# HKUST-Aerial-Robotics/A-LOAM

Measured on AMD Instinct MI355X. Metric: HDL-64 scans/sec (whole node), higher is better.
Workload: dtype f32 features / f64 solve

## Files before the change

### a-loam_amd/binding.py

```python
from __future__ import annotations

import ctypes as C
import os
import re
import subprocess

import numpy as np

from .records import *

_HERE = os.path.dirname(os.path.abspath(__file__))
_ROOT = os.path.dirname(_HERE)
LIB_PATH = os.path.join(_HERE, "lib", "libaloam_mi355x.so")
HEADER_PATH = os.path.join(_ROOT, "include", "aloam_mi355x.h")

MAP_INFO_KEYS = ("cenW", "cenH", "cenD", "frame_count", "from_map_corner", "from_map_surf", "corner_stack", "surf_stack",
                 "corner_num0", "corner_num1", "surf_num0", "surf_num1", "lm_iterations0", "lm_iterations1", "termination0", "compactions")


class AloamError(RuntimeError):
    def __init__(self, code, msg):
        super().__init__(f"aloam error {code}: {msg}")
        self.code = code

# ... 33 lines not shown
        L.aloam_create.argtypes = [C.POINTER(AloamConfig), C.POINTER(vp)]
        L.aloam_create_stages.argtypes = [C.POINTER(AloamConfig), C.c_int, C.POINTER(vp)]
        L.aloam_destroy.argtypes = [vp]; L.aloam_destroy.restype = None
        L.aloam_last_error.argtypes = [vp]; L.aloam_last_error.restype = C.c_char_p
        L.aloam_stream.argtypes = [vp]; L.aloam_stream.restype = vp
        L.aloam_synchronize.argtypes = [vp]
        L.aloam_set_voxel_sum_order.argtypes = [vp, C.c_int]
        L.aloam_scan_register.argtypes = [vp, C.POINTER(vp), ip, C.c_int]
        L.aloam_scan_register_device.argtypes = [vp, vp, C.c_longlong, ip, C.c_int]
        L.aloam_scan_register_host.argtypes = [vp, vp, C.c_longlong, ip, C.c_int]
        L.aloam_process_host.argtypes = [vp, vp, C.c_longlong, ip, C.c_int]
        L.aloam_input_consumed.argtypes = [vp]
        L.aloam_odometry_step.argtypes = [vp]
        L.aloam_process_device.argtypes = [vp, vp, C.c_longlong, ip, C.c_int]
        L.aloam_set_range_decoder.argtypes = [vp, C.POINTER(AloamRangeDecoder)]
        L.aloam_scan_register_range_device.argtypes = [vp, vp, C.c_longlong, ip]
        L.aloam_scan_register_range_host.argtypes = [vp, vp, C.c_longlong, ip]
        L.aloam_process_range_device.argtypes = [vp, vp, C.c_longlong, ip]
        L.aloam_process_range_host.argtypes = [vp, vp, C.c_longlong, ip]
        L.aloam_cloud_size.argtypes = [vp, C.c_int, C.c_int]
        L.aloam_get_cloud.argtypes = [vp, C.c_int, C.c_int, vp, C.c_int]
        L.aloam_get_pose.argtypes = [vp, C.c_int, vp, vp, vp, vp]
        L.aloam_get_odom_stats.argtypes = [vp, C.c_int, C.POINTER(AloamOdomStats)]
        L.aloam_set_features.argtypes = [vp, C.c_int, vp, C.c_int, vp, C.c_int, vp, C.c_int, vp, C.c_int]
        L.aloam_set_last.argtypes = [vp, C.c_int, vp, C.c_int, vp, C.c_int]
        L.aloam_set_state.argtypes = [vp, C.c_int, vp, vp, vp, vp]
        L.aloam_set_system_inited.argtypes = [vp, C.c_int]
        L.aloam_set_active.argtypes = [vp, vp]
        L.aloam_reset_sequences.argtypes = [vp, vp, C.c_int]
        L.aloam_set_map_frozen.argtypes = [vp, vp]
        L.aloam_score_map_corrections.argtypes = [vp, vp, C.c_int, vp, C.c_int, vp, vp]
        L.aloam_apply_map_corrections.argtypes = [vp, vp, C.c_int, vp, C.c_int, vp]
        L.aloam_map_spill_enable.argtypes = [vp, C.c_int, C.c_int]
        L.aloam_export_map_spill.argtypes = [vp, vp, C.c_int, vp, C.c_longlong, vp, C.c_longlong, vp, C.c_int]
        L.aloam_get_map_spill_info.argtypes = [vp, C.c_int, vp]
        L.aloam_atlas_load.argtypes = [vp, vp, C.c_longlong, vp, C.c_longlong]
        L.aloam_atlas_attach.argtypes = [vp, vp]
        L.aloam_atlas_info.argtypes = [vp, vp]
        L.aloam_places_enable.argtypes = [vp, C.c_int, C.c_float, C.c_float]
        L.aloam_places_add.argtypes = [vp, vp, C.c_int]
        L.aloam_places_match.argtypes = [vp, vp, C.c_int, vp, C.c_int, vp]
        L.aloam_places_export.argtypes = [vp, C.c_int, C.c_int, vp]
        L.aloam_places_load.argtypes = [vp, vp, C.c_int]
        L.aloam_places_clear.argtypes = [vp]
        L.aloam_places_info.argtypes = [vp, vp]
        L.aloam_save_sequences.argtypes = [vp, vp, C.c_int, vp, C.c_longlong, vp]
        L.aloam_load_sequences.argtypes = [vp, vp, C.c_int, vp, vp]
        L.aloam_get_ring_ranges.argtypes = [vp, C.c_int, vp, vp]
        L.aloam_get_curvature.argtypes = [vp, C.c_int, vp, C.c_int]
        L.aloam_get_labels.argtypes = [vp, C.c_int, vp, C.c_int]
        L.aloam_get_last_cloud_order.argtypes = [vp, C.c_int, vp]
        if hasattr(L, "aloam_get_solve_lds"):
            L.aloam_get_solve_lds.argtypes = [vp, vp]
        L.aloam_get_correspondences.argtypes = [vp, C.c_int, vp, C.c_int, ip, vp, vp, C.c_int, ip, vp]
        L.aloam_mapping_enable.argtypes = [vp, C.c_float, C.c_float, C.c_int]
        L.aloam_mapping_step.argtypes = [vp]
        L.aloam_mapping_set_pool_limit.argtypes = [vp, C.c_int]
        L.aloam_get_map_pool_info.argtypes = [vp, vp]
        L.aloam_set_map.argtypes = [vp, C.c_int, C.c_int, vp, vp, C.c_int, vp]
        L.aloam_set_map_frame.argtypes = [vp, C.c_int, vp, vp, vp, C.c_int]
        L.aloam_set_full_cloud.argtypes = [vp, C.c_int, vp, C.c_int]
        L.aloam_get_map_pose.argtypes = [vp, C.c_int, vp, vp, vp, vp]
        L.aloam_get_map_info.argtypes = [vp, C.c_int, vp]
        L.aloam_map_cube_counts.argtypes = [vp, C.c_int, C.c_int, vp]
        L.aloam_get_map_cube.argtypes = [vp, C.c_int, C.c_int, C.c_int, vp, C.c_int]
        L.aloam_get_map_cloud.argtypes = [vp, C.c_int, C.c_int, vp, C.c_int]
        L.aloam_export_poses.argtypes = [vp, vp]
        L.aloam_export_clouds.argtypes = [vp, vp, C.c_int, vp, C.c_longlong, vp]
        L.aloam_export_pose_information.argtypes = [vp, C.c_int, vp, C.c_int, vp]
        L.aloam_get_map_factors.argtypes = [vp, C.c_int, vp, C.c_int, ip, vp, C.c_int, ip]
        L.aloam_graph_default_options.argtypes = [C.POINTER(AloamGraphOptions)]; L.aloam_graph_default_options.restype = None
        L.aloam_graph_enable.argtypes = [vp, C.c_int, C.c_int]
        L.aloam_graph_add_nodes.argtypes = [vp, vp, C.c_int, vp]
        L.aloam_graph_add_edges.argtypes = [vp, vp, C.c_int]
        L.aloam_graph_export.argtypes = [vp, C.c_int, C.c_int, C.c_int, vp]
        L.aloam_graph_export_edges.argtypes = [vp, C.c_int, C.c_int, C.c_int, vp]
        L.aloam_graph_clear.argtypes = [vp, vp, C.c_int]
        L.aloam_graph_info.argtypes = [vp, C.c_int, vp]
        L.aloam_graph_optimize.argtypes = [vp, vp, C.c_int, C.POINTER(AloamGraphOptions), vp]
        L.aloam_graph_keyframes_enable.argtypes = [vp, C.c_int, C.c_int]
        L.aloam_graph_export_keyframes.argtypes = [vp, C.c_int, C.c_int, C.c_int, C.c_int, vp, C.c_longlong, vp]
        L.aloam_graph_keyframe_info.argtypes = [vp, C.c_int, vp]
        L.aloam_graph_export_map.argtypes = [vp, vp, C.c_int, vp, C.c_longlong, vp, C.c_longlong, vp, vp]
        L.aloam_graph_apply.argtypes = [vp, vp, C.c_int, vp]
        L.aloam_graph_loop_default_options.argtypes = [C.POINTER(AloamGraphLoopOptions)]; L.aloam_graph_loop_default_options.restype = None
        L.aloam_graph_loops_enable.argtypes = [vp, C.c_int, C.c_int, C.c_int]
        L.aloam_graph_register_loops.argtypes = [vp, vp, C.c_int, C.POINTER(AloamGraphLoopOptions), vp]
        L.aloam_graph_loop_export_target.argtypes = [vp, C.c_int, C.c_int, vp, C.c_longlong, vp]
        L.aloam_graph_loop_default_search.argtypes = [C.POINTER(AloamGraphLoopSearch)]; L.aloam_graph_loop_default_search.restype = None
        L.aloam_graph_search_loops.argtypes = [vp, vp, C.c_int, C.POINTER(AloamGraphLoopSearch), C.POINTER(AloamGraphLoopOptions), vp, vp, vp]
        L.aloam_graph_marginal_default_options.argtypes = [C.POINTER(AloamGraphMarginalOptions)]; L.aloam_graph_marginal_default_options.restype = None
        L.aloam_graph_marginals.argtypes = [vp, vp, C.c_int, C.POINTER(AloamGraphMarginalOptions), vp]
        L.aloam_graph_robust_default_options.argtypes = [C.POINTER(AloamGraphRobustOptions)]; L.aloam_graph_robust_default_options.restype = None
        L.aloam_graph_optimize_robust.argtypes = [vp, vp, C.c_int, C.POINTER(AloamGraphOptions), C.POINTER(AloamGraphRobustOptions), vp, vp, C.c_longlong]
        if hasattr(L, "aloam_graph_propose_loops"):
            L.aloam_graph_propose_loops.argtypes = [vp, vp, C.c_int, C.c_int, C.c_double, C.c_double, C.c_int, C.c_int, C.c_int, C.c_int, vp, vp, vp]
        L.aloam_graph_save.argtypes = [vp, vp, C.c_int, vp, C.c_longlong, vp]
        L.aloam_graph_load.argtypes = [vp, vp, C.c_int, vp, vp]
        L.aloam_profile_enable.argtypes = [vp, C.c_int]
        L.aloam_profile_kernel_count.argtypes = []
        L.aloam_profile_kernel_name.argtypes = [C.c_int]; L.aloam_profile_kernel_name.restype = C.c_char_p
        L.aloam_profile_get.argtypes = [vp, C.c_int, C.POINTER(C.c_double), C.POINTER(C.c_longlong), C.POINTER(C.c_double)]
        _lib = L
    return _lib


# ... 589 lines not shown

    def graph_load(self, slots, blob, offsets):
        ids = _ids(slots)
        off = np.ascontiguousarray(offsets, dtype=np.int64)
        ptr = blob.data_ptr() if hasattr(blob, "data_ptr") else blob.ctypes.data
        self._graph_load_keep = (blob, off)
        self._check(lib().aloam_graph_load(self.h, _ids_arg(ids), len(ids), _vp(ptr), _p(off)))

    def save_sequences_into(self, seqs, dst_ptr, cap_bytes, offsets_ptr):
        ids = _ids(seqs)
        self._check(lib().aloam_save_sequences(self.h, _ids_arg(ids), len(ids), _vp(dst_ptr), int(cap_bytes), _vp(offsets_ptr)))

    def save_sequences(self, seqs, pinned=True):
        import torch
        off = torch.zeros(len(seqs) + 1, dtype=torch.int64, pin_memory=True)
        self.save_sequences_into(seqs, 0, 0, off.data_ptr())
        self.synchronize()
        total = int(off[-1])
        blob = torch.empty(max(total, 16), dtype=torch.uint8, **_where(pinned))
        self.save_sequences_into(seqs, blob.data_ptr(), total, off.data_ptr())
        self.synchronize()
        return (blob[:total].numpy() if pinned else blob[:total]), off.numpy().copy()

    def load_sequences(self, slots, blob, offsets):
        ids = _ids(slots)
        off = np.ascontiguousarray(offsets, dtype=np.int64)
        ptr = blob.data_ptr() if hasattr(blob, "data_ptr") else blob.ctypes.data
        self._load_keep = (blob, off)
        self._check(lib().aloam_load_sequences(self.h, _ids_arg(ids), len(ids), _vp(ptr), _p(off)))

    def odometry_step(self):
        self._check(lib().aloam_odometry_step(self.h))

    def pose(self, seq=0):
        qw, tw, ql, tl = np.zeros(4), np.zeros(3), np.zeros(4), np.zeros(3)
        self._check(lib().aloam_get_pose(self.h, seq, _p(qw), _p(tw), _p(ql), _p(tl)))
        return {"q_w": qw, "t_w": tw, "q_lc": ql, "t_lc": tl}

    def odom_stats(self, seq=0):
        st = AloamOdomStats()
        self._check(lib().aloam_get_odom_stats(self.h, seq, C.byref(st)))
        return {k: list(getattr(st, k)) for k, _ in AloamOdomStats._fields_}

    def last_cloud_order(self, seq=0):
        v = np.zeros(2, np.int32)
        self._check(lib().aloam_get_last_cloud_order(self.h, seq, _p(v)))
        return int(v[0]), int(v[1])

    def solve_lds(self):
        v = np.zeros(3, np.int32)
        self._check(lib().aloam_get_solve_lds(self.h, _p(v)))
        return int(v[0]), int(v[1]), int(v[2])

    def correspondences(self, seq=0):
        cap_e, cap_p = self.n_scans * 12, self.n_scans * 24
        e = np.zeros((cap_e, 9), np.float32); p = np.zeros((cap_p, 12), np.float32)
        eq = np.zeros(cap_e, np.int32); pq = np.zeros(cap_p, np.int32)
        ne, npl = C.c_int(0), C.c_int(0)
        self._check(lib().aloam_get_correspondences(self.h, seq, _p(e), cap_e, C.byref(ne), _p(eq), _p(p), cap_p, C.byref(npl), _p(pq)))
        return e[:ne.value].copy(), p[:npl.value].copy(), eq[:ne.value].copy(), pq[:npl.value].copy()

    def mapping_enable(self, line_res=0.4, plane_res=0.8, pool_points=262144, pool_limit=None):
        if pool_limit is not None:
            self._check(lib().aloam_mapping_set_pool_limit(self.h, int(pool_limit)))
        self._check(lib().aloam_mapping_enable(self.h, float(line_res), float(plane_res), int(pool_points)))

    def map_pool_info(self):
        v = np.zeros(4, np.int32)
        self._check(lib().aloam_get_map_pool_info(self.h, _p(v)))
        return {"pool_points": int(v[0]), "growths": int(v[1]), "limit": int(v[2]), "live_max": int(v[3])}

    def set_map(self, cubes, cls, seq=0):
        ids = np.array(sorted(cubes), np.int32)
        cnt = np.array([len(cubes[int(i)]) for i in ids], np.int32)
        pts = _f32(np.concatenate([cubes[int(i)] for i in ids])) if len(ids) else np.zeros((0, 4), np.float32)
        self._check(lib().aloam_set_map(self.h, seq, cls, _p(ids), _p(cnt), len(ids), _p(pts)))

    def set_map_frame(self, cen, q_wmap_wodom, t_wmap_wodom, frame_count, seq=0):
        a, q, t = np.ascontiguousarray(cen, dtype=np.int32), _f64(q_wmap_wodom), _f64(t_wmap_wodom)
        self._check(lib().aloam_set_map_frame(self.h, seq, _p(a), _p(q), _p(t), int(frame_count)))

    def mapping_step(self):
        self._check(lib().aloam_mapping_step(self.h))

    def set_full_cloud(self, cloud, seq=0):
        a = _f32(cloud)
        self._check(lib().aloam_set_full_cloud(self.h, seq, _p(a), len(a)))

    def mapping_step_inputs(self, q_wodom, t_wodom, corner_last, surf_last, full_res, seq=0):
        self.set_last(corner_last, surf_last, seq)
        self.set_full_cloud(full_res, seq)
        p = self.pose(seq)
        self.set_state(p["q_lc"], p["t_lc"], q_wodom, t_wodom, seq)
        self.mapping_step()
        return self.map_pose(seq)

    def map_pose(self, seq=0):
        qw, tw, qm, tm = np.zeros(4), np.zeros(3), np.zeros(4), np.zeros(3)
        self._check(lib().aloam_get_map_pose(self.h, seq, _p(qw), _p(tw), _p(qm), _p(tm)))
        return {"q_w": qw, "t_w": tw, "q_wmap_wodom": qm, "t_wmap_wodom": tm}

    def map_info(self, seq=0):
        v = np.zeros(16, np.int32)
        self._check(lib().aloam_get_map_info(self.h, seq, _p(v)))
        return dict(zip(MAP_INFO_KEYS, (int(x) for x in v)))

# ... 61 lines not shown
```

### a-loam_amd/csrc/capi_odometry.hip

```cpp
#include <algorithm>
#include <cstring>
#include <functional>

#include "capi_internal.hpp"

namespace {

RegArgs reg_args(aloam_ctx* c, const void* d_scans, long long seq_stride, int pt_stride) {
  RegArgs a{};
  a.in = (const char*)d_scans; a.seq_stride = seq_stride; a.pt_stride = pt_stride;
  a.B = c->B; a.cap = c->cap; a.R = c->R; a.NB = c->NB;
  a.ring_from_field = c->cfg.ring_from_field; a.min_range = c->cfg.min_range;
  a.meta = c->d_meta.get(); a.slabs = c->d_slabs.get(); a.slab = c->slab; a.front_lb = c->d_front_lb.get(); a.front_ticket = c->d_front_ticket.get();
  a.ringstart = c->d_ringstart.get(); a.cloud = c->d_cloud.get(); a.curv = c->d_curv.get(); a.label = c->d_label.get();
  a.lookback = c->d_lookback.get(); a.epoch = c->reg_epoch; a.store_debug = c->debug_arrays ? 1 : 0; a.ring_ticket = c->d_ring_ticket.get();
  a.sharp = c->d_sharp.get(); a.flat = c->d_flat.get();
  for (int k = 0; k < 2; ++k) { a.less_sharp[k] = c->d_less_sharp[k].get(); a.less_flat[k] = c->d_less_flat[k].get(); }
  a.active = c->reg_mask;
  return a;
}

}

namespace aloam {
// ... 453 lines not shown
  if ((rc = ensure_dense(c))) return rc;
  HIP_TRY(c, hipStreamSynchronize(c->stream));
  if (n) HIP_TRY(c, hipMemcpy(cloud_row(c, s, seq), cloud, sizeof(float4) * n, hipMemcpyHostToDevice));
  return edit_seq(c, c->d_meta.get() + seq, [&](SeqMeta& m) { m.n_cloud = n; });
}

int aloam_get_ring_ranges(aloam_ctx* c, int seq, int* start, int* count) {
  DeviceScope device_scope(c);
  int rc = check_seq(c, seq);
  if (rc) return rc;
  if ((rc = require_stage(c, ALOAM_STAGE_REGISTRATION))) return rc;
  HIP_TRY(c, hipStreamSynchronize(c->stream));
  std::vector<int> rs(c->R + 1);
  HIP_TRY(c, hipMemcpy(rs.data(), c->d_ringstart.get() + (size_t)seq * (c->R + 1), sizeof(int) * (c->R + 1), hipMemcpyDeviceToHost));
  for (int r = 0; r < c->R; ++r) { start[r] = rs[r]; count[r] = rs[r + 1] - rs[r]; }
  return c->R;
}

int aloam_get_curvature(aloam_ctx* c, int seq, float* out, int cap) {
  DeviceScope device_scope(c);
  int rc = check_seq(c, seq);
  if (rc) return rc;
  if ((rc = require_stage(c, ALOAM_STAGE_REGISTRATION))) return rc;
  if (!c->debug_arrays) { c->err = "curvature is only kept by aloam_scan_register*; the throughput entries (aloam_process_*) skip it"; return ALOAM_E_STATE; }
  SeqMeta m;
  if ((rc = read_seq(c, c->d_meta.get() + seq, &m))) return rc;
  const int k = m.n_cloud < cap ? m.n_cloud : cap;
  if (k > 0) HIP_TRY(c, hipMemcpy(out, c->d_curv.get() + (size_t)seq * c->cap, sizeof(float) * k, hipMemcpyDeviceToHost));
  return m.n_cloud;
}

int aloam_get_labels(aloam_ctx* c, int seq, int* out, int cap) {
  DeviceScope device_scope(c);
  int rc = check_seq(c, seq);
  if (rc) return rc;
  if ((rc = require_stage(c, ALOAM_STAGE_REGISTRATION))) return rc;
  if (!c->debug_arrays) { c->err = "labels are only kept by aloam_scan_register*; the throughput entries (aloam_process_*) skip them"; return ALOAM_E_STATE; }
  SeqMeta m;
  if ((rc = read_seq(c, c->d_meta.get() + seq, &m))) return rc;
  const int k = m.n_cloud < cap ? m.n_cloud : cap;
  std::vector<int8_t> tmp(k > 0 ? k : 1);
  if (k > 0) HIP_TRY(c, hipMemcpy(tmp.data(), c->d_label.get() + (size_t)seq * c->cap, k, hipMemcpyDeviceToHost));
  for (int i = 0; i < k; ++i) out[i] = tmp[i];
  return m.n_cloud;
}

int aloam_get_solve_lds(aloam_ctx* c, int out[3]) {
  if (!c || !out) return ALOAM_E_ARG;
  if (!c->d_edges) { c->err = "this context has no odometry stage"; return ALOAM_E_STATE; }
  solve_launch_lds(odom_args(c), out);
  return ALOAM_OK;
}

int aloam_get_last_cloud_order(aloam_ctx* c, int seq, int out[2]) {
  DeviceScope device_scope(c);
  int rc = check_seq(c, seq);
  if (rc) return rc;
  if (!c->d_grid_flags[0][0]) { c->err = "this context has no odometry stage"; return ALOAM_E_STATE; }
  HIP_TRY(c, hipStreamSynchronize(c->stream));
  const int set = c->seq[seq].parity;
  for (int k = 0; k < 2; ++k) {
    int f[4];
    HIP_TRY(c, hipMemcpy(f, c->d_grid_flags[set][k].get() + (size_t)seq * 4, sizeof(f), hipMemcpyDeviceToHost));
    out[k] = f[0] ? -1 : f[1];
  }
  return ALOAM_OK;
}

int aloam_get_correspondences(aloam_ctx* c, int seq, float* edges, int cap_edges, int* n_edges, int* edge_query,
                              float* planes, int cap_planes, int* n_planes, int* plane_query) {
  DeviceScope device_scope(c);
  int rc = check_seq(c, seq);
  if (rc) return rc;
  SeqMeta m;
  if ((rc = read_seq(c, c->d_meta.get() + seq, &m))) return rc;
  std::vector<EdgeRec> E(m.n_sharp > 0 ? m.n_sharp : 1);
  std::vector<PlaneRec> P(m.n_flat > 0 ? m.n_flat : 1);
  if (m.n_sharp > 0) HIP_TRY(c, hipMemcpy(E.data(), c->d_edges.get() + (size_t)seq * c->R * kSharpPerRing, sizeof(EdgeRec) * m.n_sharp, hipMemcpyDeviceToHost));
  if (m.n_flat > 0) HIP_TRY(c, hipMemcpy(P.data(), c->d_planes.get() + (size_t)seq * c->R * kFlatPerRing, sizeof(PlaneRec) * m.n_flat, hipMemcpyDeviceToHost));
  int ne = 0, np = 0;
  for (int i = 0; i < m.n_sharp; ++i) {
    if (!E[i].valid) continue;
    if (ne < cap_edges) {
      float* o = edges + (size_t)ne * 9;
      for (int k = 0; k < 3; ++k) { o[k] = E[i].cp[k]; o[3 + k] = E[i].a[k]; o[6 + k] = E[i].b[k]; }
      if (edge_query) edge_query[ne] = i;
    }
    ++ne;
  }
  for (int i = 0; i < m.n_flat; ++i) {
    if (!P[i].valid) continue;
    if (np < cap_planes) {
      float* o = planes + (size_t)np * 12;
      for (int k = 0; k < 3; ++k) { o[k] = P[i].cp[k]; o[3 + k] = P[i].j[k]; o[6 + k] = P[i].l[k]; o[9 + k] = P[i].m[k]; }
      if (plane_query) plane_query[np] = i;
    }
    ++np;
  }
  *n_edges = ne;
  *n_planes = np;
  return ALOAM_OK;
}

}
```

### a-loam_amd/csrc/odometry_kernels.hip

```cpp
#include "aloam_device.hpp"
#include "aloam_trig.hpp"
#include "lm_device.hpp"
#include "odometry_solve_device.hpp"
#include "odometry_kernels.hpp"

namespace aloam {

#define ALOAM_PHASE(name) asm volatile("; ##PHASE " name)
#ifdef ALOAM_PHASE_CLOCK
__device__ unsigned long long g_phase_clock_odo[2][32];
#define ALOAM_BG_CLOCK(slot) do { if (threadIdx.x == 0 && blockIdx.x == 1) { atomicAdd(&g_phase_clock_odo[0][slot], (unsigned long long)__builtin_readcyclecounter()); atomicAdd(&g_phase_clock_odo[1][slot], 1ull); } } while (0)
#else
#define ALOAM_BG_CLOCK(slot) do { } while (0)
#endif
#ifdef ALOAM_ASSOC_STATS
__device__ unsigned long long g_assoc_stats[2][32];
#define ALOAM_STAT(cls, i, v) do { if ((threadIdx.x & 63) == 0) atomicAdd(&g_assoc_stats[cls][i], (unsigned long long)(v)); } while (0)
#else
#define ALOAM_STAT(cls, i, v) do { } while (0)
#endif

__device__ __forceinline__ float4 transform_to_start(const float4& p, const OdomState& st) {
  double q[4] = {st.para_q[0], st.para_q[1], st.para_q[2], st.para_q[3]};
  if (q[3] < 0.0) { q[0] = -q[0]; q[1] = -q[1]; q[2] = -q[2]; q[3] = -q[3]; }
// ... 841 lines not shown
    ALOAM_STAT(PLANE ? 1 : 0, 24 + stage, 1);
    const bool wo = PLANE ? (NEARLY ? want2 || want3 : want3) : want2, ws = PLANE && (NEARLY ? want2 || want3 : want2);
    const int lc = stage == 0 ? 0 : stage == 1 ? 3 : 4, ncell = 1 << lc, nslot = PLANE ? 5 : 4;
    const int n_look = ncell * nslot + (stage == 1 && !kOwnFirst ? nslot : 0);
    ALOAM_PHASE("ring_lookup");
    for (int lb = 0; lb < n_look; lb += W) {
      const int k = lb + l;
      int s0 = 0, cnt = 0;
      const bool centre = k >= ncell * nslot;
      const int slot = centre ? k - ncell * nslot : k >> lc;
      const bool other = slot < 4;
      if (k < n_look && (other ? wo : ws)) {
        const int key = cid - 2 + (int)((0x2819u >> (slot * 3)) & 7u);
        int ddx = 0, ddy = 0;
        float gx = 0.f, gy = 0.f;
        if (stage > 0 && !centre) {
          const CellOff2 o = kRingCells[(stage == 1 ? 0 : 8) + (k & (ncell - 1))];
          ddx = o.dx; ddy = o.dy;
          gx = axis_gap(ddx, o.ax, ax); gy = axis_gap(ddy, o.ay, ay);
        }
        const bool second = PLANE ? !other : true;
        if (key >= 0 && (gx * gx + gy * gy) * 0.999f <= (second ? lim2 : lim3)) {
          const unsigned hh = hash3(cx + ddx, cy + ddy, key) & hm;
          bucket_bounds(g.start2, hh, s0, cnt);
        }
      }
      ALOAM_PHASE("ring_sweep");
      sweep2<HALVES, kRows>(g.sorted2, last_index, s0, cnt, lane, last4, lds, [&](const float4& p, int, bool) {
        const unsigned wb = __float_as_uint(p.w);
        consider2<PLANE, NEARLY>(dist_to(p, sxy, sz), (int)(wb & kIdxMask), (int)(wb >> 20) - 1, closest, cid, t2, t3, lo, hi);
      }, nullptr, nullptr, PLANE ? 1 : 0, 8 + 4 * stage);
    }
    ALOAM_PHASE("ring_mins");
    if (!PLANE || track2) best2 = seg_min<HALVES>(t2, last4);
    if (PLANE) best3 = seg_min<HALVES>(t3, last4);
    ALOAM_PHASE("ring_bounds");
    if (stage == 2) break;
    float bound;
    if (stage == 0) bound = (1.0f - 0.01f) * fmaxf(fminf(fminf(ax.up, ax.dn), fminf(ay.up, ay.dn)) + rc, 0.f);
    else bound = ((float)stage - 0.01f) * rc;
    const float b2 = bound * bound;
    if (!none(best2)) lim2 = __uint_as_float((unsigned)(best2 >> 32));
    if (PLANE && !none(best3)) lim3 = __uint_as_float((unsigned)(best3 >> 32));
    if (!none(best2) && lim2 <= b2) want2 = false;
    if (PLANE && !none(best3) && lim3 <= b2) want3 = false;
  }
}

__device__ __forceinline__ unsigned long long read_u64(unsigned long long v, int src) {
  return ((unsigned long long)(unsigned)__builtin_amdgcn_readlane((int)(unsigned)(v >> 32), src) << 32) | (unsigned)__builtin_amdgcn_readlane((int)(unsigned)v, src);
}
__device__ __forceinline__ float read_f32(float v, int src) { return __int_as_float(__builtin_amdgcn_readlane(__float_as_int(v), src)); }

template <bool PLANE, int kRows, bool PAIRED_TAILS, bool NEARLY>
__device__ __forceinline__ void associate_pair(const OdomArgs& a, int b, int qi0, int nq, int nt, const GridView& g, int lane, int* lds) {
  constexpr int kRows1 = (kRows + 1) / 2;
  const int l = lane & 31, hsel = lane >> 5, last4 = (lane | 31) << 2;
  const int qi = qi0 + hsel;
  const bool qact = qi < nq;
  const int qcap = PLANE ? a.R * kFlatPerRing : a.R * kSharpPerRing;
  const long long qo = (long long)b * qcap + (qact ? qi : qi0);
  const float4 raw = (PLANE ? a.flat : a.sharp)[qo];
  const float4 sel = (PLANE ? a.sel_flat : a.sel_sharp)[qo];
  const float frac = raw.w - (float)(int)raw.w;
  const int parity = a.meta[b].parity;
  const float4* T = PLANE ? surf_last(a, b, parity) : corner_last(a, b, parity);
  const unsigned hm = (unsigned)(g.H - 1), last_index = (unsigned)(nt - 1);
  const float cell = cell3_of(PLANE ? 1 : 0);
  const float2v selxy = {sel.x, sel.y};

  ALOAM_PHASE("setup");
  unsigned long long t1 = ~0ull;
  KeptPair<kRows> kept;
  int kept_rows = 0;
#pragma unroll
  for (int u = 0; u < kRows; ++u) kept.k[u] = ~0ull;
  {
    const float inv = 1.0f / cell;
    const int cx = (int)floorf(sel.x * inv), cy = (int)floorf(sel.y * inv), cz = (int)floorf(sel.z * inv);
    int s0 = 0, cnt = 0;
    if (l < 27 && qact) {
      const unsigned hh = hash3(cx + l % 3 - 1, cy + (l % 9) / 3 - 1, cz + l / 9 - 1) & hm;
      bucket_bounds(g.start3, hh, s0, cnt);
    }
    sweep2<true, kRows>(g.sorted3, last_index, s0, cnt, lane, last4, lds, [&](const float4& p, int u, bool first) {
      const unsigned long long v = nn_key(dist_to(p, selxy, sel.z), __float_as_uint(p.w));
      if (first) kept.k[u] = v;
      take_min(t1, v);
    }, &kept.ok, &kept_rows, PLANE ? 1 : 0, 4);
  }
  ALOAM_PHASE("nn_min");
  unsigned long long nn = half_min_packed(t1, last4);
  float fine_b2;
  {
    const float inv = 1.0f / cell;
    const float lx = floorf(sel.x * inv) * cell, ly = floorf(sel.y * inv) * cell, lz = floorf(sel.z * inv) * cell;
    const float gap = fminf(fminf(fminf(sel.x - lx, (lx + cell) - sel.x), fminf(sel.y - ly, (ly + cell) - sel.y)), fminf(sel.z - lz, (lz + cell) - sel.z));
    const float b = (1.0f - 0.01f) * (cell + (gap > 1e-3f ? gap - 1e-3f : 0.f));
    fine_b2 = b * b;
  }
  {
    const float bound2 = fine_b2;
    const bool need1 = qact && !(nn != ~0ull && __uint_as_float((unsigned)(nn >> 32)) <= bound2);
    const unsigned long long need = __ballot(need1);
    const bool n0 = need & 1ull, n1 = (need >> 32) & 1ull;
    if (PAIRED_TAILS && n0 && n1) nn = coarse_shells<kRows1, true>(g, last_index, cell * kCell3CoarseFactor, sel.x, sel.y, sel.z, nn, need1, lane, last4, lds, PLANE ? 1 : 0);
    else if (n0 || n1) {
      const int q = n0 ? 0 : 1;
#pragma unroll
      for (int qq = 0; qq < 2; ++qq) {
        if (PAIRED_TAILS ? qq != q : !((need >> (32 * qq)) & 1ull)) continue;
        const unsigned long long r = coarse_shells<kRows1, false>(g, last_index, cell * kCell3CoarseFactor, read_f32(sel.x, 32 * qq), read_f32(sel.y, 32 * qq), read_f32(sel.z, 32 * qq),
                                                                    read_u64(nn, 32 * qq), true, lane, 0, lds, PLANE ? 1 : 0);
        if (hsel == qq) nn = r;
      }
    }
  }
  ALOAM_PHASE("classes");
  const float nnd = __uint_as_float((unsigned)(nn >> 32));
  const bool has1 = qact && nn != ~0ull && nnd < 25.0f;
  const int closest = (int)((unsigned)nn >> 12);
  const int cid = (int)((unsigned)nn & 0xfffu) - 1;
  unsigned long long best2 = ~0ull, best3 = ~0ull;
  int wlo = -1, whi = nt;
  if (NEARLY && has1) {
    const int S = a.R + 8, c = min(max(cid, 0), a.R);
    whi = g.walk[c + 3];
    wlo = c >= 3 ? g.walk[S + c - 3] : -1;
  }
  ALOAM_STAT(PLANE ? 1 : 0, 0, 1); ALOAM_STAT(PLANE ? 1 : 0, 1, (int)((__ballot(qact) & 1) + ((__ballot(qact) >> 32) & 1))); ALOAM_STAT(PLANE ? 1 : 0, 2, (int)((__ballot(has1) & 1) + ((__ballot(has1) >> 32) & 1)));
  ALOAM_STAT(PLANE ? 1 : 0, 3, (int)((__ballot(has1 && kept.ok) & 1) + ((__ballot(has1 && kept.ok) >> 32) & 1)));
  if (__ballot(has1)) {
    bool want2 = has1, want3 = PLANE && has1;
    if (__ballot(has1 && kept.ok)) {
      unsigned long long t2 = ~0ull, t3 = ~0ull;
#pragma unroll
      for (int u = 0; u < kRows; ++u) {
        if (u >= kept_rows) continue;
        const unsigned lo = (unsigned)kept.k[u];
        consider2<PLANE, NEARLY>(__uint_as_float((unsigned)(kept.k[u] >> 32)), (int)(lo >> 12), (int)(lo & 0xfffu) - 1, closest, cid, t2, t3, wlo, whi);
      }
      const bool use = has1 && kept.ok;
      best2 = half_min_packed(use ? t2 : ~0ull, last4);
      if (PLANE) best3 = half_min_packed(use ? t3 : ~0ull, last4);
      const float b2 = fine_b2;
      if (!none(best2) && __uint_as_float((unsigned)(best2 >> 32)) <= b2) want2 = false;
      if (PLANE && !none(best3) && __uint_as_float((unsigned)(best3 >> 32)) <= b2) want3 = false;
    }
    ALOAM_PHASE("ring_tail");
    const unsigned long long w2 = __ballot(want2), w3 = __ballot(want3);
    const bool r0 = (w2 | w3) & 1ull, r1 = ((w2 | w3) >> 32) & 1ull;
    if (PAIRED_TAILS && r0 && r1) ring_grid<PLANE, kRows1, true, NEARLY>(g, last_index, sel.x, sel.y, sel.z, closest, cid, want2, want3, best2, best3, lane, last4, lds, wlo, whi);
    else {
#pragma unroll
      for (int q = 0; q < 2; ++q) {
        const bool q2 = (w2 >> (32 * q)) & 1ull, q3 = (w3 >> (32 * q)) & 1ull;
        if (!(q2 || q3)) continue;
        unsigned long long r2 = read_u64(best2, 32 * q), r3 = read_u64(best3, 32 * q);
        ring_grid<PLANE, kRows1, false, NEARLY>(g, last_index, read_f32(sel.x, 32 * q), read_f32(sel.y, 32 * q), read_f32(sel.z, 32 * q), __builtin_amdgcn_readlane(closest, 32 * q),
                                                __builtin_amdgcn_readlane(cid, 32 * q), q2, q3, r2, r3, lane, 0, lds, __builtin_amdgcn_readlane(wlo, 32 * q), __builtin_amdgcn_readlane(whi, 32 * q));
        if (hsel == q) { best2 = r2; best3 = r3; }
      }
    }
  }
  ALOAM_PHASE("record");
  const bool valid = has1 && !none(best2) && (!PLANE || !none(best3));

  if (qact) {
    constexpr int kPts = PLANE ? 4 : 3;
    float* e = PLANE ? reinterpret_cast<float*>(a.planes + (long long)b * a.R * kFlatPerRing + qi) : reinterpret_cast<float*>(a.edges + (long long)b * a.R * kSharpPerRing + qi);
    if (l < kPts) {
      float x = raw.x, y = raw.y, z = raw.z;
      if (l > 0) {
        x = y = z = 0.f;
        if (valid) {
          const int j = l == 1 ? closest : index_of(l == 2 ? best2 : best3, closest);
          const float4 p = T[j];
          x = p.x; y = p.y; z = p.z;
        }
      }
      e[3 * l] = x; e[3 * l + 1] = y; e[3 * l + 2] = z;
    } else if (l == kPts) {
      int* ei = reinterpret_cast<int*>(e) + 3 * kPts;
      ei[0] = valid ? 1 : 0; ei[1] = __float_as_int(frac); ei[2] = 0;
      if (PLANE) ei[3] = 0;
    }
  }
}

template <bool PLANE, bool WIDE>
__global__ __launch_bounds__(64) void k_associate_pair(OdomArgs a) {
  constexpr int kRows = PairRows<PLANE, WIDE>::value;
  __shared__ int lds[sweep2_lds_ints<kRows>()];
  const int lane = threadIdx.x, L = blockIdx.x, xcd = L & 7, slot = L >> 3;
  const int pairs = PLANE ? a.R * (kFlatPerRing / 2) : a.R * (kSharpPerRing / 2);
  const int b = (slot / pairs) * 8 + xcd, qi0 = (slot % pairs) * 2;
  if (b >= a.B || seq_idle(a.active, b, kSeqSolve)) return;
  const SeqMeta m = a.meta[b];
  const int nq = PLANE ? m.n_flat : m.n_sharp;
  if (qi0 >= nq) return;
  const GridView g = grid_view(a, b, PLANE ? 1 : 0, m.parity ^ 1);
  const int nt = PLANE ? m.n_surf_last : m.n_corner_last;
  if (g.flags[0] != 0 || g.flags[1] != 0 || nt <= 0) return;
  associate_pair<PLANE, kRows, !WIDE, false>(a, b, qi0, nq, nt, g, lane, lds);
}

constexpr int kPairsPerWave = 8;
template <bool PLANE, bool WIDE>
__global__ __launch_bounds__(64) void k_associate_nearly(OdomArgs a) {
  constexpr int kRows = PairRows<PLANE, WIDE>::value;
  __shared__ int lds[sweep2_lds_ints<kRows>()];
  const int lane = threadIdx.x, b = blockIdx.y;
  if (seq_idle(a.active, b, kSeqSolve)) return;
  const SeqMeta m = a.meta[b];
  const GridView g = grid_view(a, b, PLANE ? 1 : 0, m.parity ^ 1);
  if (g.flags[0] != 0 || g.flags[1] != 1) return;
  const int nq = PLANE ? m.n_flat : m.n_sharp, nt = PLANE ? m.n_surf_last : m.n_corner_last;
  if (nt <= 0) return;
  for (int k = 0; k < kPairsPerWave; ++k) {
    const int qi0 = (blockIdx.x * kPairsPerWave + k) * 2;
    if (qi0 >= nq) return;
    associate_pair<PLANE, kRows, !WIDE, true>(a, b, qi0, nq, nt, g, lane, lds);
  }
}

template <bool PLANE, bool WIDE>
__global__ __launch_bounds__(256) void k_associate_flagged(OdomArgs a) {
  constexpr int kSweep = SweepRows<PLANE, WIDE>::value;
  __shared__ int rows[4][kSweep * 64];
  const int b = blockIdx.x, lane = threadIdx.x & 63, wave = threadIdx.x >> 6;
  if (seq_idle(a.active, b, kSeqSolve)) return;
  const SeqMeta m = a.meta[b];
  const GridView g = grid_view(a, b, PLANE ? 1 : 0, m.parity ^ 1);
  const int nt = PLANE ? m.n_surf_last : m.n_corner_last;
  if (!(g.flags[0] != 0 || g.flags[1] == 2 || nt <= 0)) return;
  const int nq = PLANE ? m.n_flat : m.n_sharp;
  for (int qi = wave; qi < nq; qi += 4) associate_one<PLANE, WIDE>(a, b, qi, m, g, lane, rows[wave]);
}

template <bool DISTORT>
__global__ __launch_bounds__(kSolveThreads) void k_solve(OdomArgs a) {
  const int b = blockIdx.x, tid = threadIdx.x;
  __shared__ double s_red[kSolveWaves * 28];
  if (seq_idle(a.active, b, kSeqSolve)) return;
  OdomState& st = a.state[b];
  double q[4] = {st.para_q[0], st.para_q[1], st.para_q[2], st.para_q[3]};
  double t[3] = {st.para_t[0], st.para_t[1], st.para_t[2]};

  SolveKeep keep = {a.solve_stage ? solve_stage(a.R, DISTORT) : SolveStage{0, 0, 0}, 0u, 0u};
  bool first = true;
  const LmResult lm = lm_solve_block<kSolveWaves>([&](bool, const double* qq, const double* tt, double* acc, int* ne, int* np) __attribute__((always_inline)) {
    if (first) { first = false; evaluate<true, DISTORT, 1, kSolveAhead>(a, b, qq, tt, acc, ne, np, &keep); }
    else evaluate<true, DISTORT, 2, kSolveAhead>(a, b, qq, tt, acc, ne, np, &keep);
  }, q, t, a.lm_max_iterations, s_red);
  const int n_edges = lm.n_a, n_planes = lm.n_b, iterations = lm.iterations, successful = lm.successful, termination = lm.termination;
  const double initial_cost = lm.initial_cost, cost = lm.final_cost;

  if (tid == 0) {
    if (termination == 5) {
      for (int k = 0; k < 4; ++k) q[k] = st.para_q[k];
      for (int k = 0; k < 3; ++k) t[k] = st.para_t[k];
    }
    for (int k = 0; k < 4; ++k) st.para_q[k] = q[k];
    for (int k = 0; k < 3; ++k) st.para_t[k] = t[k];
    const int o = a.outer < 2 ? a.outer : 1;
    st.corner_corr[o] = n_edges;
    st.plane_corr[o] = n_planes;
    st.lm_iterations[o] = iterations;
    st.lm_successful[o] = successful;
    st.initial_cost[o] = initial_cost;
    st.final_cost[o] = cost;
    st.termination[o] = termination;
    if (a.last_outer) {
      const double qw[4] = {st.q_w[0], st.q_w[1], st.q_w[2], st.q_w[3]};
      double rt[3];
// ... 6 lines not shown
    }
  }
}

__global__ void k_advance(SeqMeta* meta, OdomState* state, const int* active, int B) {
  const int b = blockIdx.x * blockDim.x + threadIdx.x;
  if (b >= B || seq_idle(active, b)) return;
  SeqMeta& m = meta[b];
  m.n_corner_last = m.n_less_sharp; m.n_surf_last = m.n_less_flat; m.parity ^= 1;
  state[b].inited = 1;
}
__global__ void k_set_inited(OdomState* state, int B, int inited) {
  const int b = blockIdx.x * blockDim.x + threadIdx.x;
  if (b < B) state[b].inited = inited;
}
void launch_set_inited(OdomState* state, int B, int inited, hipStream_t s) { hipLaunchKernelGGL(k_set_inited, dim3((B + 63) / 64), dim3(64), 0, s, state, B, inited); }
void launch_advance(const OdomArgs& a, hipStream_t s) { hipLaunchKernelGGL(k_advance, dim3((a.B + 63) / 64), dim3(64), 0, s, a.meta, a.state, a.active, a.B); }

size_t build_grids_lds_bytes(int H, int R) { return sizeof(int) * ((size_t)H + 1024 + 2 * (R + 8) + 4); }
static size_t build_grids_fused_lds_bytes(int H) { return sizeof(int) * (3 * (size_t)(H / 2) + 48 + 8 + 2 * kWalkKeys); }
int prepare_build_grids(int H_surf) {
  const int fused = (int)build_grids_fused_lds_bytes(kFusedMaxH), per_grid = (int)build_grids_lds_bytes(H_surf, kMaxRings);
  if (hipFuncSetAttribute((const void*)k_build_grids_fused, hipFuncAttributeMaxDynamicSharedMemorySize, fused) != hipSuccess) return -1;
  if (hipFuncSetAttribute((const void*)k_build_grids_fused_next, hipFuncAttributeMaxDynamicSharedMemorySize, fused) != hipSuccess) return -1;
  if (hipFuncSetAttribute((const void*)k_build_grids_fused_last, hipFuncAttributeMaxDynamicSharedMemorySize, fused) != hipSuccess) return -1;
  if (hipFuncSetAttribute((const void*)k_build_grids, hipFuncAttributeMaxDynamicSharedMemorySize, per_grid) != hipSuccess) return -1;
  return hipFuncSetAttribute((const void*)k_build_grids_next, hipFuncAttributeMaxDynamicSharedMemorySize, per_grid) == hipSuccess ? 0 : -1;
}
void launch_build_grids(const OdomArgs& a, GridBuild form, int wgs, hipStream_t s) {
  const int hc = a.grid_H_corner <= kFusedMaxH ? a.grid_H_corner : 0, hs = a.grid_H_surf <= kFusedMaxH ? a.grid_H_surf : 0;
  const size_t fused = build_grids_fused_lds_bytes(hc > hs ? hc : hs), per_grid = build_grids_lds_bytes(a.grid_H_surf, a.R);
  const int even = wgs >= 2 ? wgs & ~1 : 2;
  const dim3 walk(2 * a.B < even ? 2 * a.B : even);
  switch (form) {
    case GridBuild::kPersistentNext:
      if (hc || hs) hipLaunchKernelGGL(k_build_grids_fused_next, walk, dim3(1024), fused, s, a);
      hipLaunchKernelGGL(k_build_grids_next, dim3(6, a.B), dim3(1024), per_grid, s, a);
      break;
    case GridBuild::kPersistentLast:
      if (hc || hs) hipLaunchKernelGGL(k_build_grids_fused_last, walk, dim3(1024), fused, s, a);
      hipLaunchKernelGGL(k_build_grids, dim3(6, a.B), dim3(1024), per_grid, s, a);
      break;
    case GridBuild::kSerialLast:
      if (hc || hs) hipLaunchKernelGGL(k_build_grids_fused, dim3(2, a.B), dim3(1024), fused, s, a);
      hipLaunchKernelGGL(k_build_grids, dim3(6, a.B), dim3(1024), per_grid, s, a);
      break;
  }
}
void launch_transform_queries(const OdomArgs& a, hipStream_t s) {
  const dim3 grid((a.R * (kSharpPerRing + kFlatPerRing) + 255) / 256, a.B);
  if (a.distortion) hipLaunchKernelGGL(k_transform_queries<true>, grid, dim3(256), 0, s, a);
  else hipLaunchKernelGGL(k_transform_queries<false>, grid, dim3(256), 0, s, a);
}
void launch_associate(const OdomArgs& a, bool plane, hipStream_t s) {
  const int by = (a.B + 7) / 8 * 8;
  const int qcap = plane ? a.R * kFlatPerRing : a.R * kSharpPerRing;
  const bool wide = a.R > 64;
  const dim3 grid((unsigned)(qcap / 2 * by)), block(64), gridf((unsigned)a.B), blockf(256);
  const dim3 gridn((unsigned)((qcap / 2 + kPairsPerWave - 1) / kPairsPerWave), (unsigned)a.B);
  if (wide) {
    if (plane) { hipLaunchKernelGGL((k_associate_pair<true, true>), grid, block, 0, s, a); hipLaunchKernelGGL((k_associate_nearly<true, true>), gridn, block, 0, s, a); hipLaunchKernelGGL((k_associate_flagged<true, true>), gridf, blockf, 0, s, a); }
    else { hipLaunchKernelGGL((k_associate_pair<false, true>), grid, block, 0, s, a); hipLaunchKernelGGL((k_associate_nearly<false, true>), gridn, block, 0, s, a); hipLaunchKernelGGL((k_associate_flagged<false, true>), gridf, blockf, 0, s, a); }
  } else {
    if (plane) { hipLaunchKernelGGL((k_associate_pair<true, false>), grid, block, 0, s, a); hipLaunchKernelGGL((k_associate_nearly<true, false>), gridn, block, 0, s, a); hipLaunchKernelGGL((k_associate_flagged<true, false>), gridf, blockf, 0, s, a); }
    else { hipLaunchKernelGGL((k_associate_pair<false, false>), grid, block, 0, s, a); hipLaunchKernelGGL((k_associate_nearly<false, false>), gridn, block, 0, s, a); hipLaunchKernelGGL((k_associate_flagged<false, false>), gridf, blockf, 0, s, a); }
  }
}
int prepare_solve() {
  const int most = kSolveLdsBudget - kSolveStaticLds;
  if (hipFuncSetAttribute((const void*)k_solve<true>, hipFuncAttributeMaxDynamicSharedMemorySize, most) != hipSuccess) return -1;
  return hipFuncSetAttribute((const void*)k_solve<false>, hipFuncAttributeMaxDynamicSharedMemorySize, most) == hipSuccess ? 0 : -1;
}
void solve_launch_lds(const OdomArgs& a, int out[3]) {
  const SolveStage st = a.solve_stage ? solve_stage(a.R, a.distortion != 0) : SolveStage{0, 0, 0};
  out[0] = st.plane_slots; out[1] = st.edge_slots; out[2] = st.bytes;
}
void launch_solve(const OdomArgs& a, hipStream_t s) {
  int keep[3];
  solve_launch_lds(a, keep);
  const size_t lds = (size_t)keep[2];
  if (a.distortion) hipLaunchKernelGGL(k_solve<true>, dim3(a.B), dim3(kSolveThreads), lds, s, a);
  else hipLaunchKernelGGL(k_solve<false>, dim3(a.B), dim3(kSolveThreads), lds, s, a);
}
}

#ifdef ALOAM_PHASE_CLOCK
extern "C" int aloam_debug_phase_clock_odo(unsigned long long* out) { return (int)hipMemcpyFromSymbol(out, HIP_SYMBOL(aloam::g_phase_clock_odo), sizeof(unsigned long long) * 64); }
#endif
#ifdef ALOAM_ASSOC_STATS
extern "C" int aloam_debug_assoc_stats(unsigned long long* out) { return (int)hipMemcpyFromSymbol(out, HIP_SYMBOL(aloam::g_assoc_stats), sizeof(unsigned long long) * 64); }
#endif
```

### a-loam_amd/csrc/odometry_kernels.hpp

```cpp
#pragma once
#include "aloam_device.hpp"

struct aloam_pose_information;

namespace aloam {
size_t build_grids_lds_bytes(int H, int R);
int prepare_build_grids(int H_surf);
enum class GridBuild { kSerialLast, kPersistentNext, kPersistentLast };
void launch_build_grids(const OdomArgs& a, GridBuild form, int wgs, hipStream_t s);
void launch_transform_queries(const OdomArgs& a, hipStream_t s);
void launch_associate(const OdomArgs& a, bool plane, hipStream_t s);
int prepare_solve();
void solve_launch_lds(const OdomArgs& a, int out[3]);
void launch_solve(const OdomArgs& a, hipStream_t s);
void launch_advance(const OdomArgs& a, hipStream_t s);
void launch_pose_information_odom(const OdomArgs& a, const int* list, int n, aloam_pose_information* dst, hipStream_t s);
void launch_set_inited(OdomState* state, int B, int inited, hipStream_t s);
}
```

### include/aloam_mi355x.h

```cpp
#ifndef ALOAM_MI355X_H_
#define ALOAM_MI355X_H_

#ifdef __cplusplus
extern "C" {
#endif

typedef struct aloam_ctx aloam_ctx;

enum {
  ALOAM_OK = 0,
  ALOAM_E_ARG = -1,
  ALOAM_E_SCAN_LINES = -2,
  ALOAM_E_EMPTY = -3,
  ALOAM_E_CAPACITY = -4,
  ALOAM_E_HIP = -5,
  ALOAM_E_STATE = -6
};

typedef struct aloam_config {
  int n_scans;
  float min_range;
  int ring_from_field;
  int batch;
  int max_points;
// ... 345 lines not shown
int aloam_graph_marginals(aloam_ctx* ctx, const aloam_graph_marginal_request* req, int n, const aloam_graph_marginal_options* opt,
                          aloam_graph_marginal_result* dst );

enum { ALOAM_GRAPH_RECORD_MAGIC = 0x52474c41, ALOAM_GRAPH_RECORD_VERSION = 1 };
enum { ALOAM_GRAPH_PART_GRAPH = 1, ALOAM_GRAPH_PART_KEYFRAMES = 2 };
typedef struct aloam_graph_record_header {
  unsigned int magic;
  unsigned int version;
  long long bytes;
  int parts;
  int nodes, edges;
  int kf_points[2];
  int seq;
  unsigned int line_res_bits, plane_res_bits;
  int node_bytes, edge_bytes, desc_bytes, point_bytes;
  int pad[16];
} aloam_graph_record_header;
int aloam_graph_save(aloam_ctx* ctx, const int* seqs, int n, void* dst, long long cap_bytes, long long* dst_offsets );
int aloam_graph_load(aloam_ctx* ctx, const int* slots, int n, const void* src, const long long* src_offsets );

typedef struct aloam_graph_robust_options {
  int max_outer_iterations;
  int pad;
  double inlier_chi2;
  double mu_step;
  double reserved;
} aloam_graph_robust_options;
typedef struct aloam_graph_robust_result {
  aloam_graph_result solve;
  int outer_iterations, robust_edges, inliers, outliers;
  double mu, s_max, truncated_cost;
  double reserved[3];
} aloam_graph_robust_result;
void aloam_graph_robust_default_options(aloam_graph_robust_options* opt);
int aloam_graph_optimize_robust(aloam_ctx* ctx, const int* seqs, int n, const aloam_graph_options* opt, const aloam_graph_robust_options* robust,
                                aloam_graph_robust_result* dst , double* weights_dst , long long weights_stride);

int aloam_graph_propose_loops(aloam_ctx* ctx, const int* queries , int n, int pose,
                              double radius_m, double growth_m_per_node, int min_gap, int half_window, int separation, int K,
                              aloam_graph_loop_request* dst , int* counts , double* dist2 );

int aloam_get_ring_ranges(aloam_ctx* ctx, int seq, int* start, int* count);
int aloam_get_curvature(aloam_ctx* ctx, int seq, float* out, int cap);
int aloam_get_labels(aloam_ctx* ctx, int seq, int* out, int cap);
int aloam_get_correspondences(aloam_ctx* ctx, int seq, float* edges, int cap_edges, int* n_edges, int* edge_query,
                              float* planes, int cap_planes, int* n_planes, int* plane_query);
int aloam_get_map_factors(aloam_ctx* ctx, int seq, double* lines, int cap_lines, int* n_lines, double* planes, int cap_planes, int* n_planes);
int aloam_graph_loop_export_target(aloam_ctx* ctx, int slot, int feature_class, float* dst_xyzw, long long cap, int* count);

int aloam_get_last_cloud_order(aloam_ctx* ctx, int seq, int out[2]);

int aloam_get_solve_lds(aloam_ctx* ctx, int out[3]);

int aloam_profile_enable(aloam_ctx* ctx, int on);
int aloam_profile_kernel_count(void);
const char* aloam_profile_kernel_name(int kernel);
int aloam_profile_get(aloam_ctx* ctx, int kernel, double* total_ms, long long* launches, double* algorithmic_bytes);

#ifdef __cplusplus
}
#endif
#endif
```

Measured before the change: 141,800.

## Prefetch pair queries via lane loads and pack nearly-associate into 4-wave blocks

Query points for each pair are now fetched by individual lanes and broadcast with readlane. The next pair's queries are prefetched while the current pair is being associated. The per-sequence prologue (active bits, meta, grid flags) is loaded up front and tested with one combined early-exit. The nearly kernel runs 4 waves per block with per-wave LDS, which cuts block count but raises LDS per block and may lower occupancy; a plan query API is added for introspection.

New measurement: 142,300 (median of 6 runs). About the same (+0.3%).

```diff
diff --git a/a-loam_amd/binding.py b/a-loam_amd/binding.py
--- a/a-loam_amd/binding.py
+++ b/a-loam_amd/binding.py
@@ -109,6 +109,8 @@
         L.aloam_get_last_cloud_order.argtypes = [vp, C.c_int, vp]
         if hasattr(L, "aloam_get_solve_lds"):
             L.aloam_get_solve_lds.argtypes = [vp, vp]
+        if hasattr(L, "aloam_get_assoc_plan"):
+            L.aloam_get_assoc_plan.argtypes = [vp, vp]
         L.aloam_get_correspondences.argtypes = [vp, C.c_int, vp, C.c_int, ip, vp, vp, C.c_int, ip, vp]
         L.aloam_mapping_enable.argtypes = [vp, C.c_float, C.c_float, C.c_int]
         L.aloam_mapping_step.argtypes = [vp]
@@ -804,6 +806,11 @@
         self._check(lib().aloam_get_solve_lds(self.h, _p(v)))
         return int(v[0]), int(v[1]), int(v[2])
 
+    def assoc_plan(self):
+        v = np.zeros(4, np.int32)
+        self._check(lib().aloam_get_assoc_plan(self.h, _p(v)))
+        return tuple({"pair_grid": int(v[2 * k]), "nearly_x": int(v[2 * k + 1])} for k in range(2))
+
     def correspondences(self, seq=0):
         cap_e, cap_p = self.n_scans * 12, self.n_scans * 24
         e = np.zeros((cap_e, 9), np.float32); p = np.zeros((cap_p, 12), np.float32)
diff --git a/a-loam_amd/csrc/capi_odometry.hip b/a-loam_amd/csrc/capi_odometry.hip
--- a/a-loam_amd/csrc/capi_odometry.hip
+++ b/a-loam_amd/csrc/capi_odometry.hip
@@ -529,6 +529,16 @@
   return ALOAM_OK;
 }
 
+int aloam_get_assoc_plan(aloam_ctx* c, int out[4]) {
+  if (!c || !out) return ALOAM_E_ARG;
+  if (!c->d_edges) { c->err = "this context has no odometry stage"; return ALOAM_E_STATE; }
+  for (int k = 0; k < 2; ++k) {
+    const AssocPlan p = plan_associate(odom_args(c), k == 1);
+    out[2 * k] = (int)p.pair_grid; out[2 * k + 1] = (int)p.nearly_x;
+  }
+  return ALOAM_OK;
+}
+
 int aloam_get_last_cloud_order(aloam_ctx* c, int seq, int out[2]) {
   DeviceScope device_scope(c);
   int rc = check_seq(c, seq);
diff --git a/a-loam_amd/csrc/odometry_kernels.hip b/a-loam_amd/csrc/odometry_kernels.hip
--- a/a-loam_amd/csrc/odometry_kernels.hip
+++ b/a-loam_amd/csrc/odometry_kernels.hip
@@ -917,19 +917,28 @@
 }
 __device__ __forceinline__ float read_f32(float v, int src) { return __int_as_float(__builtin_amdgcn_readlane(__float_as_int(v), src)); }
 
+struct PairQueries {
+  int v;
+  __device__ __forceinline__ float raw(int h, int c) const { return __int_as_float(__builtin_amdgcn_readlane(v, 4 * h + c)); }
+  __device__ __forceinline__ float sel(int h, int c) const { return __int_as_float(__builtin_amdgcn_readlane(v, 8 + 4 * h + c)); }
+};
+template <bool PLANE>
+__device__ __forceinline__ PairQueries fetch_queries(const OdomArgs& a, int b, int qi0, int lane) {
+  const int qcap = PLANE ? a.R * kFlatPerRing : a.R * kSharpPerRing;
+  const long long qo = (long long)b * qcap + qi0;
+  const float4* src = (lane & 8) ? (PLANE ? a.sel_flat : a.sel_sharp) : (PLANE ? a.flat : a.sharp);
+  return {__hip_atomic_load(reinterpret_cast<const int*>(src + qo) + (lane & 7), __ATOMIC_RELAXED, __HIP_MEMORY_SCOPE_WAVEFRONT)};
+}
+
 template <bool PLANE, int kRows, bool PAIRED_TAILS, bool NEARLY>
-__device__ __forceinline__ void associate_pair(const OdomArgs& a, int b, int qi0, int nq, int nt, const GridView& g, int lane, int* lds) {
+__device__ __forceinline__ void associate_pair(const OdomArgs& a, int b, int qi0, int nq, int nt, const GridView& g, const float4* __restrict__ T, const PairQueries& q, int lane, int* lds) {
   constexpr int kRows1 = (kRows + 1) / 2;
   const int l = lane & 31, hsel = lane >> 5, last4 = (lane | 31) << 2;
   const int qi = qi0 + hsel;
   const bool qact = qi < nq;
-  const int qcap = PLANE ? a.R * kFlatPerRing : a.R * kSharpPerRing;
-  const long long qo = (long long)b * qcap + (qact ? qi : qi0);
-  const float4 raw = (PLANE ? a.flat : a.sharp)[qo];
-  const float4 sel = (PLANE ? a.sel_flat : a.sel_sharp)[qo];
-  const float frac = raw.w - (float)(int)raw.w;
-  const int parity = a.meta[b].parity;
-  const float4* T = PLANE ? surf_last(a, b, parity) : corner_last(a, b, parity);
+  const bool second = hsel && qact;
+  const float s0x = q.sel(0, 0), s0y = q.sel(0, 1), s0z = q.sel(0, 2), s1x = q.sel(1, 0), s1y = q.sel(1, 1), s1z = q.sel(1, 2);
+  const float4 sel = make_float4(second ? s1x : s0x, second ? s1y : s0y, second ? s1z : s0z, 0.f);
   const unsigned hm = (unsigned)(g.H - 1), last_index = (unsigned)(nt - 1);
   const float cell = cell3_of(PLANE ? 1 : 0);
   const float2v selxy = {sel.x, sel.y};
@@ -1031,9 +1040,12 @@
   ALOAM_PHASE("record");
   const bool valid = has1 && !none(best2) && (!PLANE || !none(best3));
 
+  const float r0x = q.raw(0, 0), r0y = q.raw(0, 1), r0z = q.raw(0, 2), r0w = q.raw(0, 3), r1x = q.raw(1, 0), r1y = q.raw(1, 1), r1z = q.raw(1, 2), r1w = q.raw(1, 3);
   if (qact) {
+    const float4 raw = make_float4(hsel ? r1x : r0x, hsel ? r1y : r0y, hsel ? r1z : r0z, hsel ? r1w : r0w);
     constexpr int kPts = PLANE ? 4 : 3;
     float* e = PLANE ? reinterpret_cast<float*>(a.planes + (long long)b * a.R * kFlatPerRing + qi) : reinterpret_cast<float*>(a.edges + (long long)b * a.R * kSharpPerRing + qi);
+    const float frac = raw.w - (float)(int)raw.w;
     if (l < kPts) {
       float x = raw.x, y = raw.y, z = raw.z;
       if (l > 0) {
@@ -1053,6 +1065,18 @@
   }
 }
 
+struct PairPrologue { int bits; SeqMeta m; int flag0, flag1; };
+__device__ __forceinline__ PairPrologue pair_prologue(const OdomArgs& a, int b, int which) {
+  PairPrologue p;
+  const int bits = *(a.active ? a.active + b : &a.meta[b].parity);
+  p.bits = a.active ? bits : kSeqSolve;
+  p.m = a.meta[b];
+  const int2 f0 = *reinterpret_cast<const int2*>(grid_ptr(a.grid_flags, 0, which) + b * 4), f1 = *reinterpret_cast<const int2*>(grid_ptr(a.grid_flags, 1, which) + b * 4);
+  const bool one = (p.m.parity ^ 1) != 0;
+  p.flag0 = one ? f1.x : f0.x; p.flag1 = one ? f1.y : f0.y;
+  return p;
+}
+
 template <bool PLANE, bool WIDE>
 __global__ __launch_bounds__(64) void k_associate_pair(OdomArgs a) {
   constexpr int kRows = PairRows<PLANE, WIDE>::value;
@@ -1060,32 +1084,44 @@
   const int lane = threadIdx.x, L = blockIdx.x, xcd = L & 7, slot = L >> 3;
   const int pairs = PLANE ? a.R * (kFlatPerRing / 2) : a.R * (kSharpPerRing / 2);
   const int b = (slot / pairs) * 8 + xcd, qi0 = (slot % pairs) * 2;
-  if (b >= a.B || seq_idle(a.active, b, kSeqSolve)) return;
-  const SeqMeta m = a.meta[b];
-  const int nq = PLANE ? m.n_flat : m.n_sharp;
-  if (qi0 >= nq) return;
-  const GridView g = grid_view(a, b, PLANE ? 1 : 0, m.parity ^ 1);
-  const int nt = PLANE ? m.n_surf_last : m.n_corner_last;
-  if (g.flags[0] != 0 || g.flags[1] != 0 || nt <= 0) return;
-  associate_pair<PLANE, kRows, !WIDE, false>(a, b, qi0, nq, nt, g, lane, lds);
+  if (b >= a.B) return;
+  const PairQueries q = fetch_queries<PLANE>(a, b, qi0, lane);
+  const PairPrologue pr = pair_prologue(a, b, PLANE ? 1 : 0);
+  const int nq = PLANE ? pr.m.n_flat : pr.m.n_sharp, nt = PLANE ? pr.m.n_surf_last : pr.m.n_corner_last;
+  if (!(pr.bits & kSeqSolve) | (qi0 >= nq) | (pr.flag0 != 0) | (pr.flag1 != 0) | (nt <= 0)) return;
+  const GridView g = grid_view(a, b, PLANE ? 1 : 0, pr.m.parity ^ 1);
+  const float4* T = PLANE ? surf_last(a, b, pr.m.parity) : corner_last(a, b, pr.m.parity);
+  associate_pair<PLANE, kRows, !WIDE, false>(a, b, qi0, nq, nt, g, T, q, lane, lds);
+}
+
+__device__ __forceinline__ int lane_of_pair() {
+  int l;
+  asm volatile("v_mbcnt_lo_u32_b32 %0, -1, 0\n\tv_mbcnt_hi_u32_b32 %0, -1, %0" : "=v"(l));
+  return l;
 }
 
 constexpr int kPairsPerWave = 8;
+constexpr int kNearlyWaves = 4;
 template <bool PLANE, bool WIDE>
-__global__ __launch_bounds__(64) void k_associate_nearly(OdomArgs a) {
+__global__ __launch_bounds__(64 * kNearlyWaves) void k_associate_nearly(OdomArgs a) {
   constexpr int kRows = PairRows<PLANE, WIDE>::value;
-  __shared__ int lds[sweep2_lds_ints<kRows>()];
-  const int lane = threadIdx.x, b = blockIdx.y;
-  if (seq_idle(a.active, b, kSeqSolve)) return;
-  const SeqMeta m = a.meta[b];
-  const GridView g = grid_view(a, b, PLANE ? 1 : 0, m.parity ^ 1);
-  if (g.flags[0] != 0 || g.flags[1] != 1) return;
-  const int nq = PLANE ? m.n_flat : m.n_sharp, nt = PLANE ? m.n_surf_last : m.n_corner_last;
-  if (nt <= 0) return;
-  for (int k = 0; k < kPairsPerWave; ++k) {
-    const int qi0 = (blockIdx.x * kPairsPerWave + k) * 2;
-    if (qi0 >= nq) return;
-    associate_pair<PLANE, kRows, !WIDE, true>(a, b, qi0, nq, nt, g, lane, lds);
+  __shared__ int lds[kNearlyWaves][sweep2_lds_ints<kRows>()];
+  const int wave = __builtin_amdgcn_readfirstlane(threadIdx.x >> 6), b = blockIdx.y;
+  const int pairs = PLANE ? a.R * (kFlatPerRing / 2) : a.R * (kSharpPerRing / 2);
+  const int first = (blockIdx.x * kNearlyWaves + wave) * kPairsPerWave;
+  PairQueries q = fetch_queries<PLANE>(a, b, 2 * (first < pairs ? first : pairs - 1), threadIdx.x & 63);
+  const PairPrologue pr = pair_prologue(a, b, PLANE ? 1 : 0);
+  const int nq = PLANE ? pr.m.n_flat : pr.m.n_sharp, nt = PLANE ? pr.m.n_surf_last : pr.m.n_corner_last;
+  if (!(pr.bits & kSeqSolve) | (2 * first >= nq) | (pr.flag0 != 0) | (pr.flag1 != 1) | (nt <= 0)) return;
+  const GridView g = grid_view(a, b, PLANE ? 1 : 0, pr.m.parity ^ 1);
+  const float4* T = PLANE ? surf_last(a, b, pr.m.parity) : corner_last(a, b, pr.m.parity);
+  for (int p = first;; ++p) {
+    const bool more = p + 1 < first + kPairsPerWave && 2 * (p + 1) < nq;
+    const PairQueries cur = q;
+    const int lane = lane_of_pair();
+    if (more) q = fetch_queries<PLANE>(a, b, 2 * (p + 1), lane);
+    associate_pair<PLANE, kRows, !WIDE, true>(a, b, 2 * p, nq, nt, g, T, cur, lane, lds[wave]);
+    if (!more) break;
   }
 }
 
@@ -1198,18 +1234,22 @@
   if (a.distortion) hipLaunchKernelGGL(k_transform_queries<true>, grid, dim3(256), 0, s, a);
   else hipLaunchKernelGGL(k_transform_queries<false>, grid, dim3(256), 0, s, a);
 }
+AssocPlan plan_associate(const OdomArgs& a, bool plane) {
+  const int by = (a.B + 7) / 8 * 8;
+  const int pairs = (plane ? a.R * kFlatPerRing : a.R * kSharpPerRing) / 2;
+  return {(unsigned)(pairs * by), (unsigned)((pairs + kNearlyWaves * kPairsPerWave - 1) / (kNearlyWaves * kPairsPerWave))};
+}
 void launch_associate(const OdomArgs& a, bool plane, hipStream_t s) {
-  const int by = (a.B + 7) / 8 * 8;
-  const int qcap = plane ? a.R * kFlatPerRing : a.R * kSharpPerRing;
+  const AssocPlan p = plan_associate(a, plane);
   const bool wide = a.R > 64;
-  const dim3 grid((unsigned)(qcap / 2 * by)), block(64), gridf((unsigned)a.B), blockf(256);
-  const dim3 gridn((unsigned)((qcap / 2 + kPairsPerWave - 1) / kPairsPerWave), (unsigned)a.B);
+  const dim3 grid(p.pair_grid), block(64), gridf((unsigned)a.B), blockf(256);
+  const dim3 gridn(p.nearly_x, (unsigned)a.B), blockn(64 * kNearlyWaves);
   if (wide) {
-    if (plane) { hipLaunchKernelGGL((k_associate_pair<true, true>), grid, block, 0, s, a); hipLaunchKernelGGL((k_associate_nearly<true, true>), gridn, block, 0, s, a); hipLaunchKernelGGL((k_associate_flagged<true, true>), gridf, blockf, 0, s, a); }
-    else { hipLaunchKernelGGL((k_associate_pair<false, true>), grid, block, 0, s, a); hipLaunchKernelGGL((k_associate_nearly<false, true>), gridn, block, 0, s, a); hipLaunchKernelGGL((k_associate_flagged<false, true>), gridf, blockf, 0, s, a); }
+    if (plane) { hipLaunchKernelGGL((k_associate_pair<true, true>), grid, block, 0, s, a); hipLaunchKernelGGL((k_associate_nearly<true, true>), gridn, blockn, 0, s, a); hipLaunchKernelGGL((k_associate_flagged<true, true>), gridf, blockf, 0, s, a); }
+    else { hipLaunchKernelGGL((k_associate_pair<false, true>), grid, block, 0, s, a); hipLaunchKernelGGL((k_associate_nearly<false, true>), gridn, blockn, 0, s, a); hipLaunchKernelGGL((k_associate_flagged<false, true>), gridf, blockf, 0, s, a); }
   } else {
-    if (plane) { hipLaunchKernelGGL((k_associate_pair<true, false>), grid, block, 0, s, a); hipLaunchKernelGGL((k_associate_nearly<true, false>), gridn, block, 0, s, a); hipLaunchKernelGGL((k_associate_flagged<true, false>), gridf, blockf, 0, s, a); }
-    else { hipLaunchKernelGGL((k_associate_pair<false, false>), grid, block, 0, s, a); hipLaunchKernelGGL((k_associate_nearly<false, false>), gridn, block, 0, s, a); hipLaunchKernelGGL((k_associate_flagged<false, false>), gridf, blockf, 0, s, a); }
+    if (plane) { hipLaunchKernelGGL((k_associate_pair<true, false>), grid, block, 0, s, a); hipLaunchKernelGGL((k_associate_nearly<true, false>), gridn, blockn, 0, s, a); hipLaunchKernelGGL((k_associate_flagged<true, false>), gridf, blockf, 0, s, a); }
+    else { hipLaunchKernelGGL((k_associate_pair<false, false>), grid, block, 0, s, a); hipLaunchKernelGGL((k_associate_nearly<false, false>), gridn, blockn, 0, s, a); hipLaunchKernelGGL((k_associate_flagged<false, false>), gridf, blockf, 0, s, a); }
   }
 }
 int prepare_solve() {
diff --git a/a-loam_amd/csrc/odometry_kernels.hpp b/a-loam_amd/csrc/odometry_kernels.hpp
--- a/a-loam_amd/csrc/odometry_kernels.hpp
+++ b/a-loam_amd/csrc/odometry_kernels.hpp
@@ -9,6 +9,8 @@
 enum class GridBuild { kSerialLast, kPersistentNext, kPersistentLast };
 void launch_build_grids(const OdomArgs& a, GridBuild form, int wgs, hipStream_t s);
 void launch_transform_queries(const OdomArgs& a, hipStream_t s);
+struct AssocPlan { unsigned pair_grid, nearly_x; };
+AssocPlan plan_associate(const OdomArgs& a, bool plane);
 void launch_associate(const OdomArgs& a, bool plane, hipStream_t s);
 int prepare_solve();
 void solve_launch_lds(const OdomArgs& a, int out[3]);
diff --git a/include/aloam_mi355x.h b/include/aloam_mi355x.h
--- a/include/aloam_mi355x.h
+++ b/include/aloam_mi355x.h
@@ -421,6 +421,8 @@
 
 int aloam_get_solve_lds(aloam_ctx* ctx, int out[3]);
 
+int aloam_get_assoc_plan(aloam_ctx* ctx, int out[4]);
+
 int aloam_profile_enable(aloam_ctx* ctx, int on);
 int aloam_profile_kernel_count(void);
 const char* aloam_profile_kernel_name(int kernel);
```
